# SEU-dynamical-models/Manifold-based-optical-flow-method

Hardware: AMD Instinct MI355X
Metric: flow timesteps/sec on 160k-vertex mesh (higher is better)
Workload: dtype f32

## Files before the change

### include/mof.h

```cpp
#ifndef MOF_H_
#define MOF_H_

#include <stdint.h>

#ifdef __cplusplus
extern "C" {
#endif

#define MOF_ABI_VERSION 4

#define MOF_OK 0
#define MOF_E_ARG (-1)
#define MOF_E_HIP (-2)
#define MOF_E_NOCONV (-3)
#define MOF_E_STATE (-4)

#define MOF_GEOM_F32_POINTS 1u
#define MOF_NO_REORDER 2u

#define MOF_PREC_F64 0
#define MOF_PREC_MIXED 1

#define MOF_IO_DEVICE 1u
#define MOF_NO_BLOCK_JACOBI 2u
// ... 140 lines not shown
int mof_test_force_residual_trips(int32_t on);
int mof_test_residual_launches(int64_t *counts);

int mof_assembly_probe(const int32_t *tri, int32_t N, int32_t M, uint32_t flags, int64_t *staged_bytes,
                       int32_t *staged_used);
int mof_test_force_assembly_rows(int32_t on);
int mof_test_force_assembly_trips(int32_t on);
int mof_test_assembly_launches(int64_t *counts);
int mof_test_assembly_readback(mof_mesh *mesh, int32_t system, float *A32, void *A0h, double *rhs,
                               int32_t *have_A0h);

int mof_test_amg_levels(mof_mesh *mesh, int32_t level, int32_t *n_levels, int64_t *sizes, float *omegas,
                        int32_t *sell_off, int32_t *sell_col, int32_t *sell_row, int32_t *diag_pos, uint8_t *dead,
                        int32_t *twin, int32_t *mirror, int32_t *agg, int32_t *pptr, int32_t *pcol, float *Q,
                        int32_t *gptr, int32_t *gent);
int mof_test_amg_readback(mof_mesh *mesh, int32_t level, int32_t system, float *A, uint32_t *Dh, uint16_t *Dh22,
                          uint32_t *Ah, uint16_t *Ah22, float *cinv);
int mof_test_force_galerkin_ns(int32_t on);
int mof_test_galerkin_launches(int64_t *counts);
int mof_test_amg_vcycle(mof_mesh *mesh, int32_t B, const float *r, const int32_t *smap, int32_t nl,
                        const uint8_t *retired, int32_t zh, int32_t tap, const uint32_t *sentinel, uint32_t *z,
                        double *rz, int32_t nsys, const int32_t *systems, uint32_t *r1, uint32_t *taps,
                        float *coarse, int32_t *meta);
int mof_test_amg_vcycle_tables(mof_mesh *mesh, int32_t level, int32_t system, int64_t *sizes, int32_t *apos,
                               int32_t *mptr, int32_t *mlist, int32_t *rptr, int32_t *rent, int32_t *bsw_rows,
                               int32_t *bsw_bsrc, uint32_t *bsw_A);
int mof_test_vcycle_launches(int64_t *counts);
int mof_test_pcg_inner(mof_mesh *mesh, int32_t B, const double *rhs, double rtol, double outer_rtol, double etol,
                       int32_t amg, uint32_t precision, int32_t max_iter, const uint8_t *active, int32_t *hint,
                       const uint32_t *sentinel, void *x, void *r, void *z, void *p, void *q, uint32_t *x0,
                       double *scal, int32_t *sysi, double *sysd, void *dinv, int32_t a_system, void *A,
                       int32_t *meta);
int mof_test_pcg_launches(int64_t *counts);
int mof_test_outer_readback(mof_mesh *mesh, int32_t B, double *x64, double *r64, void *xin, int32_t xin_bytes,
                            int32_t *sysi, double *sysd);

int mof_xcd_map_check(int32_t nblk, int32_t batch, int32_t group);
int mof_xcd_batch_cap(int64_t nblk, int32_t group, int32_t *batch);

typedef struct mof_dd mof_dd;

typedef struct mof_dd_info {
    int32_t nparts;
    int32_t local_parts;
    int32_t rank;
    int32_t max_neighbours;
    int32_t max_owned;
    int32_t pad_;
    int64_t ghost_rows;
    int64_t send_rows;
    double ms_setup;
} mof_dd_info;

#define MOF_DD_ID_BYTES 128

int mof_partition_rcb(const double *xyz, int32_t N, int32_t nparts, int32_t *part);

int mof_dd_plan_info(const int32_t *tri, int32_t N, int32_t M, int32_t nparts, const int32_t *part,
                     int32_t *n_own, int32_t *n_ghost, int32_t *n_nbr, int32_t *n_tri,
                     int64_t *n_send);

#define MOF_DD_STAGED 64u
int mof_dd_create(const double *xyz, const double *nrm, const int32_t *tri, const double *area,
                  int32_t N, int32_t M, int32_t nparts, const int32_t *part, int32_t device,
                  uint32_t flags, mof_dd **out);

// ... 77 lines not shown
```

### manifold-based-optical-flow-method_amd/csrc/mof_pcg.hip

```cpp
#include <algorithm>
#include <cstdio>
#include <cstdlib>
#include <chrono>
#include <cmath>
#include <memory>

#include <hip/hip_ext.h>

#include "mof_dd.h"
#include "mof_internal.h"
#include "mof_rowkern.h"
#include "mof_staged.h"

namespace mof {

thread_local double g_fetch_ms = 0.0;
thread_local int64_t g_fetch_n = 0;

enum { kPcRedPq = 16, kPcRedRzrr, kPcUpdate, kPcConvEarly, kPcOuterUpdate, kPcOuterCheck, kPcCompact, kPcKernels };
std::atomic<int64_t> g_pcg_launches[kPcKernels];

namespace {

template <typename V>
struct PcgArgs {
    int32_t N, nblk, B;
    MatArgs<V> mat;
    const V *dinv;
    V *x, *r, *z, *p, *q;
    double *part_pq;
    double *part_rzrr;
    double *sysd;
    int32_t *sysi;
    int32_t ext;
    V *x0;
    V omega;
    const uint2 *dA;
    int64_t dA_nb;
    const int32_t *dA_off;
    RedArgs red;
    int32_t stall;
    double *sc;
    int32_t zh;
    SysMap sm;
    int32_t selfred;
};

__device__ __forceinline__ double *sc_rzrr(double *sc, int32_t B, int32_t slot, int32_t b) {
    return sc + 2 * ((int64_t)slot * B + b);
}
__device__ __forceinline__ double *sc_pq(double *sc, int32_t B, int32_t slot, int32_t b) {
    return sc + 4 * (int64_t)B + (int64_t)slot * B + b;
}
// ... 329 lines not shown
template <typename V, int NT = kWG>
__device__ __forceinline__ void pcg_tol_sys(const PcgArgs<V> &a, double rtol, double outer_rtol, double etol,
                                            int32_t b) {
    __shared__ double lds[2 * (NT / 64)];
    int32_t *si = a.sysi + b * kSysStride;
    if (!si[SI_ACTIVE]) {
        if (threadIdx.x == 0) si[SI_CONV] = 0;
        return;
    }
    double v[2];
    reduce_sys<2, NT>(a.part_rzrr, a.red, a.B, b, v, lds);
    if (threadIdx.x == 0) {
        double t = rtol;
        if (outer_rtol > 0.0) {
            const double ff = a.sysd[b * kSysStride + SD_FF], rr = a.sysd[b * kSysStride + SD_RR];
            if (ff > 0.0 && rr > 0.0) {
                double need = 0.3 * outer_rtol * sqrt(ff / rr);
                const double est = a.sysd[b * kSysStride + SD_EST];
                if (etol > 0.0 && est > 0.0)
                    need = fmin(need, 0.5 * etol * a.sysd[b * kSysStride + SD_XMAX] / (kErrSafety * est));
                t = fmax(rtol, fmin(0.5, need));
            }
        }
        a.sysd[b * kSysStride + SD_TOL2] = t * t * v[1];
        a.sysd[b * kSysStride + SD_RR0] = v[1];
        a.sysd[b * kSysStride + SD_BEST] = v[1];
        si[SI_BEST_IT] = 0;
        si[SI_CONV] = -1;
    }
}
template <typename V>
__global__ __launch_bounds__(kWG) void k_pcg_tol(PcgArgs<V> a, double rtol, double outer_rtol, double etol) {
    pcg_tol_sys<V>(a, rtol, outer_rtol, etol, blockIdx.x);
}

template <typename V, bool FIRST, bool ZH = false, int NQ = 1, bool PK = false>
__device__ __forceinline__ void pcg_spmv_rows(const PcgArgs<V> &a, int32_t it, int32_t flags, int32_t rb, int32_t b) {
    constexpr int NT = kWG, RPT = kRows;
    __shared__ double lds[NQ * (NT / 64)];
    const int32_t tid = row_tid();
    const bool force = flags & kForce;
    const int32_t conv = a.sysi[b * kSysStride + SI_CONV];
    if (!force && (!a.sysi[b * kSysStride + SI_ACTIVE] || (conv >= 0 && conv != it))) return;
    const int64_t pqs = (int64_t)a.red.P * a.B * a.red.nmax;
    using V2 = typename VT<V>::V2;
    const int64_t vb = (int64_t)b * a.N;
    double cur[2];
    V alpha_prev = 0;
    double old[2] = {1.0, 1.0};
    bool self = false;
    if constexpr (NQ == 1) self = a.selfred != 0;
    if (self) {
        __shared__ double lds2[2 * (NT / 64)];
        const int64_t ps = (int64_t)a.red.P * a.B * a.red.nmax * 2;
        reduce_sys<2, NT>(a.part_rzrr + (it & 1) * ps, a.red, a.B, b, cur, lds2);
        if (!FIRST) {
            double pq1[1];
            reduce_sys<2, NT>(a.part_rzrr + ((it + 1) & 1) * ps, a.red, a.B, b, old, lds2);
            reduce_sys<1, NT>(a.part_pq + ((it + 1) & 1) * pqs, a.red, a.B, b, pq1, lds2);
            if (!force) alpha_prev = (V)(old[0] / pq1[0]);
        }
    } else {
        const double *c = sc_rzrr(a.sc, a.B, it & 1, b);
        cur[0] = c[0];
        cur[1] = c[1];
        if (!FIRST) {
            const double *o = sc_rzrr(a.sc, a.B, (it + 1) & 1, b);
            old[0] = o[0];
            old[1] = o[1];
            if (!force) alpha_prev = (V)(old[0] / *sc_pq(a.sc, a.B, (it + 1) & 1, b));
        }
    }
    if (!force && cur[1] <= a.sysd[b * kSysStride + SD_TOL2]) {
        if (!FIRST) {
#pragma unroll
            for (int r = 0; r < RPT; ++r) {
                const int32_t i = rb * kRowsPerWG + r * NT + tid;
                if (i >= a.N) break;
                const int64_t vi = vb + i;
                const V2 p0 = *reinterpret_cast<const V2 *>(a.p + 2 * vi);
                V2 xi = *reinterpret_cast<const V2 *>(a.x + 2 * vi);
                xi.x += alpha_prev * p0.x;
                xi.y += alpha_prev * p0.y;
                *reinterpret_cast<V2 *>(a.x + 2 * vi) = xi;
            }
        }
        if (rb == 0 && tid == 0 && a.sysi[b * kSysStride + SI_CONV] < 0)
            a.sysi[b * kSysStride + SI_CONV] = it;
        return;
    }
    if (!force && rb == 0 && tid == 0 && cur[1] < a.sysd[b * kSysStride + SD_BEST]) {
        a.sysd[b * kSysStride + SD_BEST] = cur[1];
        a.sysi[b * kSysStride + SI_BEST_IT] = it;
    }
    V beta = 0;
    if (!FIRST) beta = (V)(cur[0] / old[0]);
    double pq = 0.0;
#pragma unroll
    for (int r = 0; r < RPT; ++r) {
        const int32_t i = rb * kRowsPerWG + r * NT + tid;
        if (i >= a.N) break;
        V y0, y1;
        const int64_t vi = vb + i;
        V2 zi;
        const V *zb = ZH ? reinterpret_cast<const V *>(reinterpret_cast<const uint32_t *>(a.z) + vb) : a.z + 2 * vb;
        if constexpr (PK)
            spmv_row_t<kIxPack, V, ZH>(a.mat, b, i, zb, y0, y1);
        else
            spmv_row<V, ZH>(a.mat, b, i, zb, y0, y1);
        if constexpr (ZH) {
            const uint32_t h = reinterpret_cast<const uint32_t *>(a.z)[vi];
            zi = V2{bf16_lo(h), bf16_hi(h)};
        } else {
            zi = *reinterpret_cast<const V2 *>(a.z + 2 * vi);
        }
        V2 qi, pi;
// ... 166 lines not shown
            *reinterpret_cast<V2 *>(a.r + 2 * vi) = ri;
            if (!a.ext) {
                const V *d = dv[q];
                const V z0 = d[0] * ri.x + d[1] * ri.y, z1 = d[2] * ri.x + d[3] * ri.y;
                *reinterpret_cast<V2 *>(a.z + 2 * vi) = V2{z0, z1};
                if (i < a.red.nown) rz += (double)ri.x * z0 + (double)ri.y * z1;
            } else if constexpr (sizeof(V) == 4) {
                const float2 d = bf16_diag_solve(dh[q], ri.x, ri.y);
                st_x0(a.x0, vi, a.omega * d.x, a.omega * d.y);
            }
            if (i < a.red.nown) rr += (double)ri.x * ri.x + (double)ri.y * ri.y;
        }
        v[2 * q] = rz;
        v[2 * q + 1] = rr;
    }
    block_sum_q<2 * R, NQ>(v, lds);
    if (tid == 0) {
#pragma unroll
        for (int q = 0; q < R; ++q) {
            const int32_t rbk = g * R + q;
            if (rbk >= a.nblk) break;
            double *o = a.part_rzrr + ((it + 1) & 1) * ps + 2 * red_rec(a.red, a.B, b, rbk);
            o[0] = v[2 * q];
            o[1] = v[2 * q + 1];
        }
    }
}
template <typename V>
__global__ __launch_bounds__(kWG) void k_pcg_update(PcgArgs<V> a, int32_t it) {
    pcg_update_rows<V>(a, it, blockIdx.x, sm_b(a.sm, blockIdx.y));
}

template <typename V, int NQ = 1>
__device__ __forceinline__ void outer_update_rows(int32_t N, int32_t first, const V *__restrict__ xin,
                                                  const int32_t *__restrict__ sysi, double *__restrict__ x64,
                                                  const RedArgs &rdx, int32_t B, double *__restrict__ part_dx,
                                                  int32_t blk, int32_t b) {
    __shared__ double lds[8 * NQ];
    if (!sysi[b * kSysStride + SI_ACTIVE]) return;
    const int32_t i = blk * kWG + row_tid();
    double v[2] = {0.0, 0.0};
    if (i < N) {
        const int64_t vi = (int64_t)b * N + i;
        using V2 = typename VT<V>::V2;
        const V2 d = *reinterpret_cast<const V2 *>(xin + 2 * vi);
        double2 x = first ? make_double2(0.0, 0.0) : *reinterpret_cast<const double2 *>(x64 + 2 * vi);
        x.x += (double)d.x;
        x.y += (double)d.y;
        *reinterpret_cast<double2 *>(x64 + 2 * vi) = x;
        if (i < rdx.nown) {
            v[0] = fmax(fabs((double)d.x), fabs((double)d.y));
            v[1] = fmax(fabs(x.x), fabs(x.y));
        }
    }
    block_max_q<2, NQ>(v, lds);
    if (row_tid() == 0 && blk < rdx.nmax) {
        double *o = part_dx + 2 * red_rec(rdx, B, b, blk);
        o[0] = v[0];
        o[1] = v[1];
    }
}
template <typename V>
__global__ __launch_bounds__(kWG) void k_outer_update(int32_t N, int32_t first, const V *__restrict__ xin,
                                                      const int32_t *__restrict__ sysi, double *__restrict__ x64,
                                                      RedArgs rdx, int32_t B, double *__restrict__ part_dx) {
    outer_update_rows<V>(N, first, xin, sysi, x64, rdx, B, part_dx, blockIdx.x, blockIdx.y);
}

template <int NQ = 1>
__device__ __forceinline__ void residual_rows(const OpArgs<double> &op, int32_t B, const RedArgs &rd,
                                              const double *__restrict__ rhs, const double *__restrict__ x64,
                                              const int32_t *__restrict__ sysi, double *__restrict__ r64,
                                              double *__restrict__ part, int32_t rb, int32_t b) {
    __shared__ double lds[8 * NQ];
    const int32_t tid = row_tid();
    if (!sysi[b * kSysStride + SI_ACTIVE]) return;
    const int32_t N = op.N;
    const int64_t vb = (int64_t)b * N;
    double rr = 0.0, ff = 0.0;
#pragma unroll
    for (int r = 0; r < kRows; ++r) {
        const int32_t i = rb * kRowsPerWG + r * kWG + tid;
        if (i >= N) break;
        double y0, y1;
        apply_row_mf<double>(op, b, i, x64 + 2 * vb, y0, y1);
        const double2 f = *reinterpret_cast<const double2 *>(rhs + 2 * (vb + i));
        const double r0 = f.x - y0, r1 = f.y - y1;
        *reinterpret_cast<double2 *>(r64 + 2 * (vb + i)) = make_double2(r0, r1);
        if (i < rd.nown) {
            rr += r0 * r0 + r1 * r1;
            ff += f.x * f.x + f.y * f.y;
        }
    }
    double v[2] = {rr, ff};
    block_sum_q<2, NQ>(v, lds);
    if (tid == 0 && rb < rd.nmax) {
        double *o = part + 2 * red_rec(rd, B, b, rb);
        o[0] = v[0];
        o[1] = v[1];
// ... 497 lines not shown
constexpr double kCompactFrac = 0.9;
constexpr int32_t kBulkHint = 48;
constexpr double kBulkFrac = 0.9;

inline int32_t sys_iters(const int32_t *si, int32_t it) {
    if (si[SI_CONV] >= 0) return si[SI_CONV];
    return si[SI_FAILED] && si[SI_FAIL_WHY] != FW_MAXITER ? si[SI_FAIL_IT] + 1 : it;
}

void charge_chunk(const mof_mesh *m, int32_t B, const std::vector<int32_t> &running_at, int32_t it0,
                  int32_t n, uint32_t precision, int32_t solve_systems, const std::vector<float> &ms,
                  SpmvTiming *t) {
    std::vector<int32_t> active(n, 0);
    for (int32_t b = 0; b < B; ++b) {
        if (!running_at[b]) continue;
        const int32_t last = sys_iters(m->h_sysi + b * kSysStride, it0 + n);
        for (int32_t c = 0; c < n && it0 + c < last; ++c) active[c]++;
    }
    for (int32_t c = 0; c < n; ++c) {
        t->ms += ms[c];
        t->launches++;
        t->systems += active[c];
        if (active[c]) t->bytes += spmv_launch_bytes(m, precision, active[c]);
        if (active[c] == solve_systems) {
            t->full_launches++;
            t->ms_full += ms[c];
        }
    }
}

template <typename V>
int64_t pcg(Parts<V> &p, const double *const *rhs, double rtol, const SolveParams &sp, hipStream_t s,
            int32_t *max_iters, SpmvTiming *timing, int32_t *hint, bool amg, double outer_rtol = 0.0,
            double etol = 0.0) {
    const int32_t max_iter = sp.max_iter, B = p.B;
    const size_t L = p.mesh.size();
    mof_mesh *mh = p.host;
    std::vector<PcgArgs<V>> &args = p.args;
    const bool single = p.d == nullptr;
    const bool compact = single;
    const bool selfred = single && args[0].red.P == 1 && args[0].nblk <= kSelfRedBlk;
    const bool early = amg && single;
    bool zh = false;
    if constexpr (sizeof(V) == 4) zh = amg && single && amg_fine(p.mesh[0]).regular;
    const bool bulk_hint = single;
    const bool timed = timing && single;
    if (!single) outer_rtol = etol = 0.0;
    for (PcgArgs<V> &a : args) {
        a.sm = sys_all(B);
        a.selfred = selfred;
        a.zh = zh;
    }
    const int64_t rec = (int64_t)B * p.nmax;
    const int64_t pqs = p.P * rec, ps = 2 * pqs;
    auto cycles = [&](int32_t slot) {
        if constexpr (sizeof(V) == 4)
            for (size_t l = 0; l < L; ++l)
                amg_vcycle(p.mesh[l], B, args[l].r, args[l].z, p.part_rzrr + slot * ps, args[l].nblk, args[l].red, s,
                           zh, args[l].sm.map, args[l].sm.n);
    };
    auto sync_rzrr = [&](int32_t slot) { p.sync(p.part_rzrr + slot * ps, 2 * rec, s); };
    auto red_rzrr = [&](int32_t slot) {
        if (selfred) return;
        for (size_t l = 0; l < L; ++l) {
            ++g_pcg_launches[kPcRedRzrr];
            k_red_rzrr<V><<<dim3((unsigned)args[l].sm.n), kWG, 0, s>>>(args[l], slot);
        }
    };
    auto red_pq = [&](int32_t slot) {
        if (selfred) return;
        for (size_t l = 0; l < L; ++l) {
            ++g_pcg_launches[kPcRedPq];
            k_red_pq<V><<<dim3((unsigned)args[l].sm.n), kWG, 0, s>>>(args[l], slot);
        }
    };
// ... 15 lines not shown
    for (int32_t b = 0; b < B; ++b) {
        was_active[b] = mh->h_sysi[b * kSysStride + SI_ACTIVE];
        solve_systems += was_active[b];
    }
    running_at = was_active;
    std::vector<int32_t> h_map(B);
    auto cover = [&](int32_t n) {
        int32_t *smap = p.mesh[0]->ws.smap.p;
        MOF_HIP(hipMemcpyAsync(smap, h_map.data(), sizeof(int32_t) * n, hipMemcpyHostToDevice, s));
        args[0].sm = SysMap{smap, n};
        ++g_pcg_launches[kPcCompact];
    };
    if (compact && solve_systems <= kCompactFrac * B) {
        int32_t n = 0;
        for (int32_t b = 0; b < B; ++b)
            if (was_active[b]) h_map[n++] = b;
        if (n > 0) cover(n);
    }
    for (size_t l = 0; l < L; ++l)
        k_pcg_init<V><<<dim3((unsigned)args[l].nblk, (unsigned)B), kWG, 0, s>>>(args[l], rhs[l]);
    sync_rzrr(0);
    for (size_t l = 0; l < L; ++l) k_pcg_tol<V><<<dim3((unsigned)B), kWG, 0, s>>>(args[l], rtol, outer_rtol, etol);
    if (amg) {
        cycles(0);
        sync_rzrr(0);
    }
    red_rzrr(0);
    MOF_HIP(hipGetLastError());
    int32_t it = 0;
    const int32_t bulk = bulk_hint ? hint[kBulkHint] : 0;
    const bool split = bulk > 0 && *hint >= bulk + 2;
    int32_t chunk = split ? std::min(bulk, kMaxChunk) : (*hint > 0 ? std::min(*hint, kMaxChunk) : 8);
    bool done = false;
    std::vector<hipEvent_t> &ev = mh->spmv_events;
    std::vector<float> ms;
    while (!done && it < max_iter) {
        const int32_t n = std::min(chunk, max_iter - it);
        if (timed && (int32_t)ev.size() < 2 * n) {
            const size_t old = ev.size();
            ev.resize(2 * (size_t)std::max(n, 64));
            for (size_t q = old; q < ev.size(); ++q) MOF_HIP(hipEventCreate(&ev[q]));
        }
        const int32_t it0 = it;
        for (int32_t c = 0; c < n; ++c, ++it) {
            if (timed)
                spmv(it == 0, it, ev[2 * c], ev[2 * c + 1]);
            else
                spmv(it == 0, it);
            red_pq(it & 1);
            for (const PcgArgs<V> &a : args) {
                ++g_pcg_launches[kPcUpdate];
                k_pcg_update<V><<<dim3(upd_blocks(a.nblk), (unsigned)a.sm.n), kWG, 0, s>>>(a, it);
            }
            for (size_t l = 0; early && l < L; ++l) {
                ++g_pcg_launches[kPcConvEarly];
                k_pcg_conv_early<V><<<dim3((unsigned)args[l].sm.n), kWG, 0, s>>>(args[l], it);
            }
            if (amg) cycles((it + 1) & 1);
            sync_rzrr((it + 1) & 1);
            red_rzrr((it + 1) & 1);
        }
        MOF_HIP(hipGetLastError());
        fetch_flags(mh, B, s);
        if (timed) {
            ms.assign(n, 0.f);
            for (int32_t c = 0; c < n; ++c) MOF_HIP(hipEventElapsedTime(&ms[c], ev[2 * c], ev[2 * c + 1]));
            charge_chunk(mh, B, running_at, it0, n, sp.precision, solve_systems, ms, timing);
        }
        done = true;
        int32_t owe_or_run = 0;
        for (int32_t b = 0; b < B; ++b) {
            const int32_t *si = mh->h_sysi + b * kSysStride;
            running_at[b] = si[SI_ACTIVE] && !si[SI_FAILED] && si[SI_CONV] < 0;
            if (running_at[b]) done = false;
            if (was_active[b] && !si[SI_FAILED] && (si[SI_CONV] < 0 || si[SI_CONV] >= it)) h_map[owe_or_run++] = b;
        }
        chunk = split && it == std::min(bulk, kMaxChunk) && *hint > it ? std::min(*hint - it, kMaxChunk) : 8;
        if (compact && !done && owe_or_run <= kCompactFrac * B) cover(owe_or_run);
    }
    if (!done) {
        spmv(it == 0, it);
        if (!single) red_pq(it & 1);
        if (sp.fail_at_max_iter)
            for (const PcgArgs<V> &a : args)
                k_fail_running<<<dim3((unsigned)((B + 63) / 64)), 64, 0, s>>>(B, it, a.sysi);
        MOF_HIP(hipGetLastError());
        fetch_flags(mh, B, s);
    } else if (early) {
        bool owe = false;
        for (int32_t b = 0; b < B && !owe; ++b)
            owe = was_active[b] && mh->h_sysi[b * kSysStride + SI_CONV] == it;
        if (owe) spmv(false, it);
        MOF_HIP(hipGetLastError());
    }
    int64_t total = 0;
    int32_t slowest = 0, slowest_conv = 0;
    std::vector<int32_t> convs;
    for (int32_t b = 0; b < B; ++b) {
        if (!was_active[b]) continue;
        const int32_t *si = mh->h_sysi + b * kSysStride;
        const int32_t c = si[SI_CONV], its = sys_iters(si, it);
        total += its;
        slowest = std::max(slowest, its);
        if (c >= 0) {
            slowest_conv = std::max(slowest_conv, c);
            if (bulk_hint) convs.push_back(c);
        }
    }
    if (!convs.empty()) {
        const size_t k = std::min(convs.size() - 1, (size_t)(kBulkFrac * (double)convs.size()));
        std::nth_element(convs.begin(), convs.begin() + k, convs.end());
        hint[kBulkHint] = convs[k];
    }
    *max_iters = std::max(*max_iters, slowest);
    if (slowest_conv > 0) *hint = std::min(slowest_conv + (early ? 0 : 1), kMaxChunk);
    return total;
}

struct OmegaScope {
    const std::vector<mof_mesh *> &mesh;
    std::vector<float> old;
    OmegaScope(const std::vector<mof_mesh *> &ms, float om, bool use) : mesh(ms) {
        if (use && om > 0.f)
            for (mof_mesh *m : mesh) old.push_back(amg_set_omega(m, om));
    }
// ... 20 lines not shown
        for (int k = 0; k < kSysStride; ++k) si[k] = 0;
        si[SI_ACTIVE] = 1;
        si[SI_CONV] = -1;
    }
    if (only)
        for (mof_mesh *q : p.mesh)
            MOF_HIP(hipMemcpyAsync(q->ws.sysi.p, mh->h_sysi, sizeof(int32_t) * kSysStride * B, hipMemcpyHostToDevice,
                                   s));
    if (d) {
        MOF_HIP(hipMemsetAsync(d->part_pq.p, 0, d->part_pq.bytes(), s));
        MOF_HIP(hipMemsetAsync(d->part_rzrr.p, 0, d->part_rzrr.bytes(), s));
        MOF_HIP(hipMemsetAsync(d->part_rr0.p, 0, d->part_rr0.bytes(), s));
        MOF_HIP(hipMemsetAsync(d->part_dx.p, 0, d->part_dx.bytes(), s));
    }
    bool amg = sp.amg && f32;
    for (size_t l = 0; l < L && amg; ++l) amg = amg_build(p.mesh[l]);
    if (amg)
        for (mof_mesh *q : p.mesh) {
            amg_ensure(q, B);
            if (!only) amg_setup_batch(q, B, s);
        }
    OmegaScope omega_scope(p.mesh, sp.amg_omega, amg);
    p.fill_args(amg, sp.stall);
    std::vector<int32_t> &hints = mh->iter_hint;
    const size_t nhint = d ? 2 * 16 : 2 * kBulkHint;
    if (hints.size() < nhint) hints.assign(nhint, 0);
    const int32_t hint0 = !f32 ? 0 : (d || amg ? 16 : 32);
    std::vector<const double *> rhs(L);
    int64_t iters = 0, iters_before = 0;
    int32_t o = 0;
    static const bool verbose = knob(Knob::Verbose) != nullptr;
    for (; o < sp.max_outer; ++o) {
        for (size_t l = 0; l < L; ++l) rhs[l] = o == 0 ? p.mesh[l]->ws.rhs.p : p.mesh[l]->ws.r64.p;
        iters += pcg<V>(p, rhs.data(), !f32 && o == 0 ? 0.5 * sp.rtol : sp.inner_rtol, sp, s, max_iters, tm,
                        &hints[hint0 + std::min(o, 15)], amg, o > 0 && sp.adaptive_inner ? sp.rtol : 0.0, sp.etol);
        for (size_t l = 0; l < L; ++l) {
            mof_mesh *q = p.mesh[l];
            Workspace &w = q->ws;
            const dim3 gv((unsigned)((q->N + kWG - 1) / kWG), (unsigned)B);
            ++g_pcg_launches[kPcOuterUpdate];
            k_outer_update<V><<<gv, kWG, 0, s>>>(q->N, o == 0, p.args[l].x, w.sysi.p, w.x64.p, p.rdx[l], B, p.part_dx);
        }
        p.sync(p.part_dx, 2 * (size_t)B * p.nvmax, s);
        p.halo(1, s);
        for (size_t l = 0; l < L; ++l) {
            Workspace &w = p.mesh[l]->ws;
            launch_residual(p.mesh[l], w.nblk, B, s, p.rd[l], w.rhs.p, w.x64.p, w.sysi.p, w.r64.p, p.part_rr0);
        }
        p.sync(p.part_rr0, 2 * (size_t)B * p.nmax, s);
        for (size_t l = 0; l < L; ++l) {
            Workspace &w = p.mesh[l]->ws;
            RedArgs rd = p.rd[l], rdx = p.rdx[l];
            if (d) rd.nown = rdx.nown = 0;
            ++g_pcg_launches[kPcOuterCheck];
            k_outer_check<<<dim3((unsigned)B), kWG, 0, s>>>(rd, B, p.part_rr0, rdx, p.part_dx, o == 0, sp.rtol,
                                                            sp.etol, w.sysd.p, w.sysi.p);
        }
        MOF_HIP(hipGetLastError());
        fetch_flags(mh, B, s);
        bool any = false;
        for (int32_t b = 0; b < B; ++b) any |= mh->h_sysi[b * kSysStride + SI_ACTIVE] != 0;
        if (verbose) {
            double worst = 0.0, west = 0.0;
            int32_t act = 0;
            for (int32_t b = 0; b < B; ++b) {
                const double *sd = mh->h_sysd + b * kSysStride;
                worst = std::max(worst, sd[SD_REL]);
                if (sd[SD_XMAX] > 0.0) west = std::max(west, sd[SD_EST] / sd[SD_XMAX]);
                act += mh->h_sysi[b * kSysStride + SI_ACTIVE] != 0;
            }
            std::fprintf(stderr,
                         "[mof solve] B=%d outer %d: %lld inner its (sum), max rel residual %.3e, max error est %.3e "
                         "of max|V|, %d still active\n",
                         B, o, (long long)(iters - iters_before), worst, west, act);
// ... 582 lines not shown
        if (precision == MOF_PREC_MIXED)
            mof::test_pcg_inner<float>(m, B, rhs, rtol, outer_rtol, etol, amg != 0, max_iter, active, hint, sentinel, x,
                                       r, z, p, q, x0, scal, sysi, sysd, dinv, a_system, A, meta);
        else
            mof::test_pcg_inner<double>(m, B, rhs, rtol, outer_rtol, etol, amg != 0, max_iter, active, hint, sentinel,
                                        x, r, z, p, q, x0, scal, sysi, sysd, dinv, a_system, A, meta);
    });
}

int mof_dd_test_pcg_inner(mof_dd *d, int32_t B, const double *rhs, double rtol, int32_t amg, uint32_t precision,
                          int32_t max_iter, const uint32_t *sentinel, void *x, void *r, void *z, void *p, void *q,
                          int32_t *sysi, double *sysd, void *dinv, int32_t a_system, void *A, double *part_rzrr,
                          double *part_pq, double *scal, int32_t *meta) {
    return mof_io_guard([&] {
        MOF_REQUIRE(d && rhs, "NULL argument");
        MOF_REQUIRE(precision == MOF_PREC_MIXED || precision == MOF_PREC_F64, "bad precision");
        mof::PcgDeviceGuard dg(d->device);
        if (precision == MOF_PREC_MIXED)
            mof::test_pcg_dd_inner<float>(d, B, rhs, rtol, amg != 0, max_iter, sentinel, x, r, z, p, q, sysi, sysd,
                                          dinv, a_system, A, part_rzrr, part_pq, scal, meta);
        else
            mof::test_pcg_dd_inner<double>(d, B, rhs, rtol, amg != 0, max_iter, sentinel, x, r, z, p, q, sysi, sysd,
                                           dinv, a_system, A, part_rzrr, part_pq, scal, meta);
    });
}

int mof_test_pcg_launches(int64_t *counts) {
    return mof_io_guard([&] {
        MOF_REQUIRE(counts, "NULL argument");
        for (int k = 0; k < mof::kPcKernels; ++k) counts[k] = mof::g_pcg_launches[k].load();
    });
}

int mof_test_outer_readback(mof_mesh *m, int32_t B, double *x64, double *r64, void *xin, int32_t xin_bytes,
                            int32_t *sysi, double *sysd) {
    return mof_io_guard([&] {
        MOF_REQUIRE(m, "mesh is NULL");
        mof::mesh_join_prep(m);
        mof::Workspace &w = m->ws;
        MOF_REQUIRE(B >= 1 && B <= w.cap, "the handle's last batch had fewer systems");
        MOF_REQUIRE(!xin || xin_bytes == 4 || xin_bytes == 8, "the inner x holds floats or doubles");
        mof::PcgDeviceGuard dg(m->device);
        MOF_HIP(hipStreamSynchronize(m->stream));
        const size_t nv = (size_t)m->N * B;
        auto get = [&](void *dst, const void *src, size_t bytes) {
            if (dst) MOF_HIP(hipMemcpy(dst, src, bytes, hipMemcpyDeviceToHost));
        };
        get(x64, w.x64.p, sizeof(double) * 2 * nv);
        get(r64, w.r64.p, sizeof(double) * 2 * nv);
        get(xin, w.vx.p, (size_t)xin_bytes * 2 * nv);
        get(sysi, w.sysi.p, sizeof(int32_t) * mof::kSysStride * B);
        get(sysd, w.sysd.p, sizeof(double) * mof::kSysStride * B);
    });
}

}
```

### manifold-based-optical-flow-method_amd/mofhip/_lib.py

```python
from __future__ import annotations

import ctypes
import os
import subprocess
import threading

import numpy as np

PKG_DIR = os.path.dirname(os.path.abspath(__file__))
ROOT_DIR = os.path.dirname(PKG_DIR)
CSRC_DIR = os.path.join(ROOT_DIR, "csrc")
LIB_PATH = os.environ.get("MOFHIP_LIB") or os.path.join(PKG_DIR, "libmofhip.so")

MOF_ABI_VERSION = 4

MOF_OK = 0
MOF_E_ARG = -1
MOF_E_HIP = -2
MOF_E_NOCONV = -3
MOF_E_STATE = -4

MOF_GEOM_F32_POINTS = 1
MOF_NO_REORDER = 2
MOF_PREC_F64 = 0
# ... 3 lines not shown
MOF_TIME_SPMV = 4
MOF_PRECOND_AMG = 8
MOF_NO_RECOVERY = 16
MOF_SOLVE_FUSED = 128
MOF_SOLVE_EAGER = 256
MOF_CSV_ROUND_TRIP = 1
MOF_COORDS_F32 = 32
MOF_DD_STAGED = 64
MOF_WAVE_PHASE = 512
MOF_WIND_ALL_LEVELS = 1024
MOF_MODES_COMPLEX = 2048
MOF_RBF_ANGLE = 4096
MOF_CSR_A2 = 0
MOF_CSR_A_LAST = 1

EXPORTS = (
    "mof_version", "mof_abi_version", "mof_last_error", "mof_device_count", "mof_mesh_create", "mof_mesh_clone",
    "mof_mesh_destroy", "mof_mesh_get_info", "mof_geometry_export", "mof_csr_export",
    "mof_assemble", "mof_solve_range", "mof_bench_spmv", "mof_velocity_vectors",
    "mof_csv_write", "mof_csv_shape", "mof_csv_read", "mof_ply_info", "mof_ply_read",
    "mof_point_normals", "mof_cell_areas", "mof_singularities", "mof_amg_probe",
    "mof_partition_rcb", "mof_dd_plan_info", "mof_dd_create", "mof_dd_unique_id",
    "mof_dd_create_rank", "mof_dd_destroy", "mof_dd_get_info", "mof_dd_solve_range",
    "mof_dd_test_fail_recovery_alloc", "mof_mesh_prepare", "mof_mesh_sync",
    "mof_singularities_compact", "mof_xcd_map_check", "mof_xcd_batch_cap", "mof_dd_create_rank_host",
    "mof_index_probe", "mof_test_force_index32", "mof_wave_speed", "mof_streamline_map", "mof_streamlines",
    "mof_test_streamline_pass", "mof_residual_probe", "mof_test_force_residual_rows",
    "mof_test_force_residual_trips", "mof_test_residual_launches", "mof_assembly_probe",
    "mof_test_force_assembly_rows", "mof_test_force_assembly_trips", "mof_test_assembly_launches",
    "mof_test_assembly_readback", "mof_winding_rings", "mof_winding_levels", "mof_winding_map",
    "mof_test_winding_pass", "mof_winding_timing", "mof_closest_vertices",
    "mof_test_amg_levels", "mof_test_amg_readback", "mof_test_force_galerkin_ns", "mof_test_galerkin_launches",
    "mof_test_amg_vcycle", "mof_test_amg_vcycle_tables", "mof_test_vcycle_launches",
    "mof_test_pcg_inner", "mof_test_pcg_launches", "mof_test_outer_readback",
    "mof_modes_gram", "mof_modes_project", "mof_test_modes_chunk", "mof_test_modes_pass",
    "mof_dd_test_part", "mof_dd_test_halo", "mof_dd_test_gather", "mof_dd_test_launches",
    "mof_dd_test_pcg_inner", "mof_rbf_eval", "mof_test_rbf_pass",
    "mof_geodesic", "mof_geodesic_edges", "mof_test_geodesic_pass", "mof_test_geodesic_tile",
    "mof_geodesic_timing", "mof_geodesic_counters",
)


class MofError(RuntimeError):

    def __init__(self, code, msg):
        super().__init__("libmofhip error %d: %s" % (code, msg))
        self.code = code


class NotConverged(MofError):
    pass


class MofOpts(ctypes.Structure):
    _fields_ = [
        ("struct_size", ctypes.c_uint32), ("precision", ctypes.c_uint32),
        ("flags", ctypes.c_uint32), ("batch", ctypes.c_int32), ("max_iter", ctypes.c_int32),
        ("max_outer", ctypes.c_int32), ("rtol", ctypes.c_double),
        ("inner_rtol", ctypes.c_double), ("stream", ctypes.c_void_p),
        ("etol", ctypes.c_double),
    ]


class MofStats(ctypes.Structure):
    _fields_ = [
        ("systems", ctypes.c_int64), ("iterations", ctypes.c_int64),
        ("max_iterations", ctypes.c_int32), ("failed", ctypes.c_int32),
# ... 104 lines not shown
            "mof_test_modes_chunk": ([i32], ctypes.c_int),
            "mof_test_modes_pass": ([i32], ctypes.c_int),
            "mof_rbf_eval": ([i32, P, i32, P, i32, f64, P, P, i32, u32, P, P, P], ctypes.c_int),
            "mof_test_rbf_pass": ([i32], ctypes.c_int),
            "mof_geodesic": ([P, P, i32, P, i32, f64, u32, P, P], ctypes.c_int),
            "mof_geodesic_edges": ([P, i64, P, P, P, P], ctypes.c_int),
            "mof_test_geodesic_pass": ([i32], ctypes.c_int),
            "mof_test_geodesic_tile": ([i32], ctypes.c_int),
            "mof_geodesic_timing": ([P], ctypes.c_int),
            "mof_geodesic_counters": ([P], ctypes.c_int),
            "mof_singularities": ([i32, P, P, i32, i32, P, i32, f64, u32, P, P, P, P, P],
                                  ctypes.c_int),
            "mof_amg_probe": ([P, P, i32, i32, P, P, P, P], ctypes.c_int),
            "mof_index_probe": ([P, i32, i32, u32, i32, P, P, P, P, P, P, P], ctypes.c_int),
            "mof_test_force_index32": ([i32], ctypes.c_int),
            "mof_residual_probe": ([P, i32, i32, u32, P, P], ctypes.c_int),
            "mof_test_force_residual_rows": ([i32], ctypes.c_int),
            "mof_test_force_residual_trips": ([i32], ctypes.c_int),
            "mof_test_residual_launches": ([P], ctypes.c_int),
            "mof_assembly_probe": ([P, i32, i32, u32, P, P], ctypes.c_int),
            "mof_test_force_assembly_rows": ([i32], ctypes.c_int),
            "mof_test_force_assembly_trips": ([i32], ctypes.c_int),
            "mof_test_assembly_launches": ([P], ctypes.c_int),
            "mof_test_assembly_readback": ([P, i32, P, P, P, P], ctypes.c_int),
            "mof_test_amg_levels": ([P, i32] + [P] * 16, ctypes.c_int),
            "mof_test_amg_readback": ([P, i32, i32, P, P, P, P, P, P], ctypes.c_int),
            "mof_test_force_galerkin_ns": ([i32], ctypes.c_int),
            "mof_test_galerkin_launches": ([P], ctypes.c_int),
            "mof_test_amg_vcycle": ([P, i32, P, P, i32, P, i32, i32, P, P, P, i32, P, P, P, P, P], ctypes.c_int),
            "mof_test_amg_vcycle_tables": ([P, i32, i32] + [P] * 9, ctypes.c_int),
            "mof_test_vcycle_launches": ([P], ctypes.c_int),
            "mof_test_pcg_inner": ([P, i32, P, f64, f64, f64, i32, u32, i32] + [P] * 13 + [i32, P, P], ctypes.c_int),
            "mof_test_pcg_launches": ([P], ctypes.c_int),
            "mof_test_outer_readback": ([P, i32, P, P, P, i32, P, P], ctypes.c_int),
            "mof_xcd_map_check": ([i32, i32, i32], ctypes.c_int),
            "mof_xcd_batch_cap": ([i64, i32, P], ctypes.c_int),
            "mof_singularities_compact": ([i32, P, P, i32, i32, P, i32, f64, u32, P, i64, P, P, P, P, P,
                                           P, P], ctypes.c_int),
            "mof_partition_rcb": ([P, i32, i32, P], ctypes.c_int),
            "mof_dd_plan_info": ([P, i32, i32, i32, P, P, P, P, P, P], ctypes.c_int),
            "mof_dd_create": ([P, P, P, P, i32, i32, i32, P, i32, u32, P], ctypes.c_int),
            "mof_dd_unique_id": ([P], ctypes.c_int),
            "mof_dd_create_rank": ([P, P, P, P, i32, i32, i32, P, i32, P, i32, u32, P],
                                   ctypes.c_int),
            "mof_dd_create_rank_host": ([P, P, P, P, i32, i32, i32, P, i32, P, i32, u32, P],
                                        ctypes.c_int),
            "mof_dd_destroy": ([P], ctypes.c_int),
            "mof_dd_get_info": ([P, P], ctypes.c_int),
            "mof_mesh_prepare": ([P, P], ctypes.c_int),
            "mof_mesh_sync": ([P], ctypes.c_int),
            "mof_dd_test_fail_recovery_alloc": ([P, i32], ctypes.c_int),
            "mof_dd_solve_range": ([P, P, P, P, i32, i32, i32, f64, P, P, P], ctypes.c_int),
            "mof_dd_test_part": ([P, i32] + [P] * 9, ctypes.c_int),
            "mof_dd_test_halo": ([P, i32, i32, i32, P, P, P], ctypes.c_int),
            "mof_dd_test_gather": ([P, i32, P, P, P, P], ctypes.c_int),
            "mof_dd_test_launches": ([P], ctypes.c_int),
            "mof_dd_test_pcg_inner": ([P, i32, P, f64, i32, u32, i32] + [P] * 9 + [i32] + [P] * 5, ctypes.c_int),
        }
        for name, (args, res) in sig.items():
            if os.environ.get("MOFHIP_LIB") and not hasattr(L, name):
                continue
            fn = getattr(L, name)
            fn.argtypes = args
            fn.restype = res
        if not os.environ.get("MOFHIP_LIB"):
            abi = L.mof_abi_version() if hasattr(L, "mof_abi_version") else 1
# ... 29 lines not shown
```

### manifold-based-optical-flow-method_amd/mofhip/mesh.py

```python
from __future__ import annotations

import ctypes
import threading
import time

import numpy as np

from . import _lib as L


def _f64(a):
    return np.ascontiguousarray(a, dtype=np.float64)


class DeviceMesh:

    def __init__(self, coordinates, normals, triangles, areas, device: int = 0,
                 reorder: bool = True):
        coords = np.asarray(coordinates)
        tri = np.asarray(triangles)
        if coords.ndim != 2 or coords.shape[1] != 3:
            raise ValueError("coordinates must be (N, 3)")
        if tri.ndim != 2 or tri.shape[1] != 3:
            raise ValueError("triangles must be (M, 3)")
# ... 230 lines not shown

def index_probe(triangles, n_vertices: int, sym: int = -1, reorder: bool = True) -> dict:
    T = np.ascontiguousarray(triangles, dtype=np.int32)
    N, M = int(n_vertices), len(T)
    flags = 0 if reorder else L.MOF_NO_REORDER
    nb, su, pu = ctypes.c_int64(0), ctypes.c_int32(0), ctypes.c_int32(0)
    L.check(L.lib().mof_index_probe(L.ptr(T), N, M, flags, int(sym), ctypes.byref(nb), None, None, None, None,
                                    None, None))
    off = np.zeros((N + 63) // 64 + 1, dtype=np.int32)
    col = np.zeros(nb.value, dtype=np.int32)
    mir = np.zeros(nb.value, dtype=np.int32)
    packed = np.zeros(nb.value, dtype=np.uint32)
    L.check(L.lib().mof_index_probe(L.ptr(T), N, M, flags, int(sym), ctypes.byref(nb), L.ptr(off), L.ptr(col),
                                    L.ptr(mir), L.ptr(packed), ctypes.byref(su), ctypes.byref(pu)))
    return {"sell_off": off, "col": col, "mir": mir, "packed": packed, "sym_used": bool(su.value),
            "packed_used": bool(pu.value)}


class _Hook:

    def __enter__(self):
        L.check(getattr(L.lib(), self._name)(1))
        return self

    def __exit__(self, *exc):
        L.check(getattr(L.lib(), self._name)(0))
        return False


class force_index32(_Hook):
    _name = "mof_test_force_index32"


def _staged_probe(name: str, triangles, n_vertices: int, reorder: bool) -> dict:
    T = np.ascontiguousarray(triangles, dtype=np.int32)
    flags = 0 if reorder else L.MOF_NO_REORDER
    nb, used = ctypes.c_int64(0), ctypes.c_int32(0)
    L.check(getattr(L.lib(), name)(L.ptr(T), int(n_vertices), len(T), flags, ctypes.byref(nb), ctypes.byref(used)))
    return {"staged_bytes": int(nb.value), "staged_used": bool(used.value)}


def _staged_launches(name: str) -> dict:
    c = np.zeros(3, dtype=np.int64)
    L.check(getattr(L.lib(), name)(L.ptr(c)))
    return {"rows": int(c[0]), "staged_one": int(c[1]), "staged_multi": int(c[2])}


def residual_probe(triangles, n_vertices: int, reorder: bool = True) -> dict:
    return _staged_probe("mof_residual_probe", triangles, n_vertices, reorder)


class force_residual_rows(_Hook):
    _name = "mof_test_force_residual_rows"


class force_residual_trips(_Hook):
    _name = "mof_test_force_residual_trips"


def residual_launches() -> dict:
    return _staged_launches("mof_test_residual_launches")


def assembly_probe(triangles, n_vertices: int, reorder: bool = True) -> dict:
    return _staged_probe("mof_assembly_probe", triangles, n_vertices, reorder)

# ... 254 lines not shown
```

Before: 4290.

## Fold owed final x update into outer update and skip trailing AMG cycle

When the inner PCG finishes, the leftover x += alpha*p step (the owed update) is no longer issued as an extra spmv launch. It is passed to the outer-update kernel, which recomputes alpha and applies it while it accumulates x64. The convergence flags are now fetched before the last chunk iteration's AMG cycle and rz/rr reduction, so that work is skipped when no system is still running. This removes a kernel launch and a V-cycle at each inner-solve seam, at the cost of an earlier host sync inside the chunk loop. A test hook is added to force the old behaviour.

Measured after the change: 4341 (median of 6 runs). +1.2%, better.

```diff
diff --git a/include/mof.h b/include/mof.h
--- a/include/mof.h
+++ b/include/mof.h
@@ -196,6 +196,7 @@
                        double *scal, int32_t *sysi, double *sysd, void *dinv, int32_t a_system, void *A,
                        int32_t *meta);
 int mof_test_pcg_launches(int64_t *counts);
+int mof_test_force_old_seams(int32_t on);
 int mof_test_outer_readback(mof_mesh *mesh, int32_t B, double *x64, double *r64, void *xin, int32_t xin_bytes,
                             int32_t *sysi, double *sysd);
 
diff --git a/manifold-based-optical-flow-method_amd/csrc/mof_pcg.hip b/manifold-based-optical-flow-method_amd/csrc/mof_pcg.hip
--- a/manifold-based-optical-flow-method_amd/csrc/mof_pcg.hip
+++ b/manifold-based-optical-flow-method_amd/csrc/mof_pcg.hip
@@ -19,6 +19,7 @@
 
 enum { kPcRedPq = 16, kPcRedRzrr, kPcUpdate, kPcConvEarly, kPcOuterUpdate, kPcOuterCheck, kPcCompact, kPcKernels };
 std::atomic<int64_t> g_pcg_launches[kPcKernels];
+std::atomic<int> g_force_old_seams{0};
 
 namespace {
 
@@ -414,6 +415,30 @@
 template <typename V>
 __global__ __launch_bounds__(kWG) void k_pcg_tol(PcgArgs<V> a, double rtol, double outer_rtol, double etol) {
     pcg_tol_sys<V>(a, rtol, outer_rtol, etol, blockIdx.x);
+}
+
+template <typename V2, typename V>
+__device__ __forceinline__ void owed_x(V alpha, const V2 &p0, V2 &xi) {
+    if constexpr (sizeof(V) == 4) {
+        xi.x = fmaf(alpha, p0.x, xi.x);
+        xi.y = fmaf(alpha, p0.y, xi.y);
+    } else {
+        xi.x += alpha * p0.x;
+        xi.y += alpha * p0.y;
+    }
+}
+template <typename V, int NT = kWG>
+__device__ __forceinline__ V owed_alpha(const PcgArgs<V> &a, int32_t it, int32_t b) {
+    const int32_t slot = (it + 1) & 1;
+    if (a.selfred) {
+        __shared__ double lds2[2 * (NT / 64)];
+        const int64_t pqs = (int64_t)a.red.P * a.B * a.red.nmax;
+        double old[2], pq1[1];
+        reduce_sys<2, NT>(a.part_rzrr + slot * 2 * pqs, a.red, a.B, b, old, lds2);
+        reduce_sys<1, NT>(a.part_pq + slot * pqs, a.red, a.B, b, pq1, lds2);
+        return (V)(old[0] / pq1[0]);
+    }
+    return (V)(sc_rzrr(a.sc, a.B, slot, b)[0] / *sc_pq(a.sc, a.B, slot, b));
 }
 
 template <typename V, bool FIRST, bool ZH = false, int NQ = 1, bool PK = false>
@@ -462,8 +487,7 @@
                 const int64_t vi = vb + i;
                 const V2 p0 = *reinterpret_cast<const V2 *>(a.p + 2 * vi);
                 V2 xi = *reinterpret_cast<const V2 *>(a.x + 2 * vi);
-                xi.x += alpha_prev * p0.x;
-                xi.y += alpha_prev * p0.y;
+                owed_x(alpha_prev, p0, xi);
                 *reinterpret_cast<V2 *>(a.x + 2 * vi) = xi;
             }
         }
@@ -696,10 +720,10 @@
 }
 
 template <typename V, int NQ = 1>
-__device__ __forceinline__ void outer_update_rows(int32_t N, int32_t first, const V *__restrict__ xin,
+__device__ __forceinline__ void outer_update_rows(int32_t N, int32_t first, V *xin,
                                                   const int32_t *__restrict__ sysi, double *__restrict__ x64,
                                                   const RedArgs &rdx, int32_t B, double *__restrict__ part_dx,
-                                                  int32_t blk, int32_t b) {
+                                                  int32_t blk, int32_t b, const V *p = nullptr, V alpha = 0) {
     __shared__ double lds[8 * NQ];
     if (!sysi[b * kSysStride + SI_ACTIVE]) return;
     const int32_t i = blk * kWG + row_tid();
@@ -707,7 +731,11 @@
     if (i < N) {
         const int64_t vi = (int64_t)b * N + i;
         using V2 = typename VT<V>::V2;
-        const V2 d = *reinterpret_cast<const V2 *>(xin + 2 * vi);
+        V2 d = *reinterpret_cast<const V2 *>(xin + 2 * vi);
+        if (p) {
+            owed_x(alpha, *reinterpret_cast<const V2 *>(p + 2 * vi), d);
+            *reinterpret_cast<V2 *>(xin + 2 * vi) = d;
+        }
         double2 x = first ? make_double2(0.0, 0.0) : *reinterpret_cast<const double2 *>(x64 + 2 * vi);
         x.x += (double)d.x;
         x.y += (double)d.y;
@@ -725,10 +753,17 @@
     }
 }
 template <typename V>
-__global__ __launch_bounds__(kWG) void k_outer_update(int32_t N, int32_t first, const V *__restrict__ xin,
-                                                      const int32_t *__restrict__ sysi, double *__restrict__ x64,
-                                                      RedArgs rdx, int32_t B, double *__restrict__ part_dx) {
-    outer_update_rows<V>(N, first, xin, sysi, x64, rdx, B, part_dx, blockIdx.x, blockIdx.y);
+__global__ __launch_bounds__(kWG) void k_outer_update(PcgArgs<V> a, int32_t first, int32_t owe,
+                                                      double *__restrict__ x64, RedArgs rdx,
+                                                      double *__restrict__ part_dx) {
+    const int32_t b = blockIdx.y;
+    const V *p = nullptr;
+    V alpha = 0;
+    if (owe >= 0 && a.sysi[b * kSysStride + SI_ACTIVE] && a.sysi[b * kSysStride + SI_CONV] == owe) {
+        p = a.p;
+        alpha = owed_alpha<V>(a, owe, b);
+    }
+    outer_update_rows<V>(a.N, first, a.x, a.sysi, x64, rdx, a.B, part_dx, blockIdx.x, b, p, alpha);
 }
 
 template <int NQ = 1>
@@ -1292,7 +1327,9 @@
 template <typename V>
 int64_t pcg(Parts<V> &p, const double *const *rhs, double rtol, const SolveParams &sp, hipStream_t s,
             int32_t *max_iters, SpmvTiming *timing, int32_t *hint, bool amg, double outer_rtol = 0.0,
-            double etol = 0.0) {
+            double etol = 0.0, int32_t *owed = nullptr) {
+    if (owed) *owed = -1;
+    const bool old_seams = g_force_old_seams.load() != 0;
     const int32_t max_iter = sp.max_iter, B = p.B;
     const size_t L = p.mesh.size();
     mof_mesh *mh = p.host;
@@ -1301,6 +1338,7 @@
     const bool compact = single;
     const bool selfred = single && args[0].red.P == 1 && args[0].nblk <= kSelfRedBlk;
     const bool early = amg && single;
+    const bool look_early = early && !old_seams;
     bool zh = false;
     if constexpr (sizeof(V) == 4) zh = amg && single && amg_fine(p.mesh[0]).regular;
     const bool bulk_hint = single;
@@ -1382,6 +1420,7 @@
     const bool split = bulk > 0 && *hint >= bulk + 2;
     int32_t chunk = split ? std::min(bulk, kMaxChunk) : (*hint > 0 ? std::min(*hint, kMaxChunk) : 8);
     bool done = false;
+    bool no_rzrr = false;
     std::vector<hipEvent_t> &ev = mh->spmv_events;
     std::vector<float> ms;
     while (!done && it < max_iter) {
@@ -1392,6 +1431,7 @@
             for (size_t q = old; q < ev.size(); ++q) MOF_HIP(hipEventCreate(&ev[q]));
         }
         const int32_t it0 = it;
+        bool looked = false;
         for (int32_t c = 0; c < n; ++c, ++it) {
             if (timed)
                 spmv(it == 0, it, ev[2 * c], ev[2 * c + 1]);
@@ -1406,12 +1446,26 @@
                 ++g_pcg_launches[kPcConvEarly];
                 k_pcg_conv_early<V><<<dim3((unsigned)args[l].sm.n), kWG, 0, s>>>(args[l], it);
             }
+            if (look_early && c == n - 1) {
+                MOF_HIP(hipGetLastError());
+                fetch_flags(mh, B, s);
+                looked = true;
+                bool running = false;
+                for (int32_t b = 0; b < B && !running; ++b) {
+                    const int32_t *si = mh->h_sysi + b * kSysStride;
+                    running = si[SI_ACTIVE] && !si[SI_FAILED] && si[SI_CONV] < 0;
+                }
+                if (!running) {
+                    no_rzrr = true;
+                    continue;
+                }
+            }
             if (amg) cycles((it + 1) & 1);
             sync_rzrr((it + 1) & 1);
             red_rzrr((it + 1) & 1);
         }
         MOF_HIP(hipGetLastError());
-        fetch_flags(mh, B, s);
+        if (!looked) fetch_flags(mh, B, s);
         if (timed) {
             ms.assign(n, 0.f);
             for (int32_t c = 0; c < n; ++c) MOF_HIP(hipEventElapsedTime(&ms[c], ev[2 * c], ev[2 * c + 1]));
@@ -1440,7 +1494,12 @@
         bool owe = false;
         for (int32_t b = 0; b < B && !owe; ++b)
             owe = was_active[b] && mh->h_sysi[b * kSysStride + SI_CONV] == it;
-        if (owe) spmv(false, it);
+        if (owe && owed && !old_seams) {
+            *owed = it;
+        } else if (owe) {
+            if (no_rzrr) red_rzrr(it & 1);
+            spmv(false, it);
+        }
         MOF_HIP(hipGetLastError());
     }
     int64_t total = 0;
@@ -1527,14 +1586,16 @@
     static const bool verbose = knob(Knob::Verbose) != nullptr;
     for (; o < sp.max_outer; ++o) {
         for (size_t l = 0; l < L; ++l) rhs[l] = o == 0 ? p.mesh[l]->ws.rhs.p : p.mesh[l]->ws.r64.p;
+        int32_t owed = -1;
         iters += pcg<V>(p, rhs.data(), !f32 && o == 0 ? 0.5 * sp.rtol : sp.inner_rtol, sp, s, max_iters, tm,
-                        &hints[hint0 + std::min(o, 15)], amg, o > 0 && sp.adaptive_inner ? sp.rtol : 0.0, sp.etol);
+                        &hints[hint0 + std::min(o, 15)], amg, o > 0 && sp.adaptive_inner ? sp.rtol : 0.0, sp.etol,
+                        &owed);
         for (size_t l = 0; l < L; ++l) {
             mof_mesh *q = p.mesh[l];
             Workspace &w = q->ws;
             const dim3 gv((unsigned)((q->N + kWG - 1) / kWG), (unsigned)B);
             ++g_pcg_launches[kPcOuterUpdate];
-            k_outer_update<V><<<gv, kWG, 0, s>>>(q->N, o == 0, p.args[l].x, w.sysi.p, w.x64.p, p.rdx[l], B, p.part_dx);
+            k_outer_update<V><<<gv, kWG, 0, s>>>(p.args[l], o == 0, owed, w.x64.p, p.rdx[l], p.part_dx);
         }
         p.sync(p.part_dx, 2 * (size_t)B * p.nvmax, s);
         p.halo(1, s);
@@ -2183,6 +2244,10 @@
     });
 }
 
+int mof_test_force_old_seams(int32_t on) {
+    return mof_io_guard([&] { mof::g_force_old_seams.store(on != 0); });
+}
+
 int mof_test_outer_readback(mof_mesh *m, int32_t B, double *x64, double *r64, void *xin, int32_t xin_bytes,
                             int32_t *sysi, double *sysd) {
     return mof_io_guard([&] {
diff --git a/manifold-based-optical-flow-method_amd/mofhip/_lib.py b/manifold-based-optical-flow-method_amd/mofhip/_lib.py
--- a/manifold-based-optical-flow-method_amd/mofhip/_lib.py
+++ b/manifold-based-optical-flow-method_amd/mofhip/_lib.py
@@ -59,7 +59,7 @@
     "mof_test_winding_pass", "mof_winding_timing", "mof_closest_vertices",
     "mof_test_amg_levels", "mof_test_amg_readback", "mof_test_force_galerkin_ns", "mof_test_galerkin_launches",
     "mof_test_amg_vcycle", "mof_test_amg_vcycle_tables", "mof_test_vcycle_launches",
-    "mof_test_pcg_inner", "mof_test_pcg_launches", "mof_test_outer_readback",
+    "mof_test_pcg_inner", "mof_test_pcg_launches", "mof_test_outer_readback", "mof_test_force_old_seams",
     "mof_modes_gram", "mof_modes_project", "mof_test_modes_chunk", "mof_test_modes_pass",
     "mof_dd_test_part", "mof_dd_test_halo", "mof_dd_test_gather", "mof_dd_test_launches",
     "mof_dd_test_pcg_inner", "mof_rbf_eval", "mof_test_rbf_pass",
@@ -230,6 +230,7 @@
             "mof_test_vcycle_launches": ([P], ctypes.c_int),
             "mof_test_pcg_inner": ([P, i32, P, f64, f64, f64, i32, u32, i32] + [P] * 13 + [i32, P, P], ctypes.c_int),
             "mof_test_pcg_launches": ([P], ctypes.c_int),
+            "mof_test_force_old_seams": ([i32], ctypes.c_int),
             "mof_test_outer_readback": ([P, i32, P, P, P, i32, P, P], ctypes.c_int),
             "mof_xcd_map_check": ([i32, i32, i32], ctypes.c_int),
             "mof_xcd_batch_cap": ([i64, i32, P], ctypes.c_int),
diff --git a/manifold-based-optical-flow-method_amd/mofhip/mesh.py b/manifold-based-optical-flow-method_amd/mofhip/mesh.py
--- a/manifold-based-optical-flow-method_amd/mofhip/mesh.py
+++ b/manifold-based-optical-flow-method_amd/mofhip/mesh.py
@@ -286,6 +286,10 @@
     _name = "mof_test_force_index32"
 
 
+class force_old_seams(_Hook):
+    _name = "mof_test_force_old_seams"
+
+
 def _staged_probe(name: str, triangles, n_vertices: int, reorder: bool) -> dict:
     T = np.ascontiguousarray(triangles, dtype=np.int32)
     flags = 0 if reorder else L.MOF_NO_REORDER
```
